# psipred/DMPfold2

Measured on AMD Instinct MI355X. Metric: structures/s at L=300, N_seq=2000, 10 iters+100 min, higher is better.
Workload: dtype f32 with full-width operands on the bf16 matrix cores (option precision = 2): convolution operands split exactly into 3 bf16 pieces (24 significand bits), the 6 piece products above 2^-24 accumulated in f32 by v_mfma_f32_32x32x16_bf16; vertical GRU the same way (3 bf16 pieces per operand, 6 products

## Files before the change

### dmpfold2_amd/csrc/conv_f16.h

```cpp
#pragma once
#include "common.h"
#include <cmath>
#include <vector>

namespace dmp {

typedef float ch_f32x16 __attribute__((ext_vector_type(16)));
typedef _Float16 ch_f16x8 __attribute__((ext_vector_type(8)));

#ifndef CH_PITCH_N
#define CH_PITCH_N 24
#endif
constexpr int CH_PITCH = CH_PITCH_N;
template <int NQ> struct ChShape {
  static constexpr int ROWS = 2 * NQ;
  static constexpr int HALO = ROWS + 4;
  static constexpr int RP = ROWS + 3;
  static constexpr int IN_SLOTS = 2 * 2 * HALO * CH_PITCH;
  static constexpr int IN_BYTES = IN_SLOTS * 16;
  static constexpr int PIECE = 2 * HALO * CH_PITCH;
};
constexpr int CH_HCOLS = 20;
constexpr int CH_WSLOT = 2 * 2 * 32;
constexpr int CH_WCOL = 5 * CH_WSLOT;
constexpr int CH_WBUF = 3 * CH_WSLOT;
template <int NQ> constexpr int convh_lds_bytes() { return ChShape<NQ>::IN_BYTES + 4 * CH_WBUF * 16; }
constexpr int CONVH_LDS_BYTES = convh_lds_bytes<8>();
inline int conv_split_rows(int tiles) { return 8 * tiles * tiles <= 256 ? 2 : 1; }
inline int conv_f16_grid(int tiles, int bands = 1) {
  const int nt = tiles * tiles * bands;
  return 8 * ((nt + 1) / 2);
}

__host__ __device__ inline uint16_t ch_f16_bits(float f) {
  const _Float16 h = (_Float16)f;
  return __builtin_bit_cast(uint16_t, h);
}
__host__ __device__ inline float ch_f16_f32(uint16_t b) {
  return (float)__builtin_bit_cast(_Float16, b);
}
__host__ __device__ inline void split2_f16(float x, uint16_t p[2]) {
  p[0] = ch_f16_bits(x);
  p[1] = ch_f16_bits(x - ch_f16_f32(p[0]));
}

inline float conv_weight_scale_f16(const float* w, size_t n) {
  float m = 0.f;
  for (size_t i = 0; i < n; ++i) m = std::fmax(m, std::fabs(w[i]));
  if (!(m > 0.f)) return 1.f;
  int e;
  std::frexp(m, &e);
  return std::ldexp(1.0f, 10 - e);
}

inline std::vector<uint16_t> pack_conv_weights_f16(const float* w, float scale) {
  const int tap_row[5] = {0, 2, 4, 1, 3};
  std::vector<uint16_t> q((size_t)4 * 8 * 25 * 4 * 2 * 2 * 32 * 8);
  for (int split = 0; split < 4; ++split)
    for (int g = 0; g < 8; ++g)
      for (int dx = 0; dx < 5; ++dx)
        for (int wave = 0; wave < 4; ++wave)
          for (int sl = 0; sl < 5; ++sl)
            for (int cg = 0; cg < 2; ++cg)
              for (int m = 0; m < 32; ++m)
                for (int e = 0; e < 8; ++e) {
                  const int oc = split * 128 + wave * 32 + m, ic = g * 16 + cg * 8 + e;
                  uint16_t p2[2];
                  split2_f16(scale * w[((size_t)oc * 128 + ic) * 25 + tap_row[sl] * 5 + dx], p2);
                  for (int p = 0; p < 2; ++p)
                    q[(((((((((size_t)split * 8 + g) * 5 + dx) * 4 + wave) * 5 + sl) * 2 + p) * 2 + cg) * 32 + m) * 8) + e] = p2[p];
                }
  return q;
}

#if defined(__HIPCC__) && defined(CONV_F16_KERNELS)
__device__ __forceinline__ void ch_dma16(const void* gsrc, unsigned lds_byte_addr) {
  unsigned keep;
  asm volatile("s_mov_b32 %0, m0\n\ts_mov_b32 m0, %2\n\ts_nop 0\n\tglobal_load_lds_dwordx4 %1, off\n\ts_mov_b32 m0, %0"
               : "=&s"(keep) : "v"(gsrc), "s"(lds_byte_addr) : "memory");
}
template <int N> __device__ __forceinline__ void ch_wait_vm() {
  asm volatile("s_waitcnt vmcnt(%0)" :: "n"(N) : "memory");
}
__device__ __forceinline__ ch_f32x16 ch_mfma(uint4 a, uint4 b, ch_f32x16 c) {
  return __builtin_amdgcn_mfma_f32_32x32x16_f16(__builtin_bit_cast(ch_f16x8, a),
                                                __builtin_bit_cast(ch_f16x8, b), c, 0, 0, 0);
}
__device__ __forceinline__ void ch_lane_pixel(int li, int& row, int& x) {
  const bool a = li < 4 || (li >= 12 && li < 16) || (li >= 20 && li < 28);
  row = a ? 0 : 1;
  if (a) x = li < 4 ? li : (li < 16 ? li - 8 : li - 12);
  else x = li < 12 ? li - 4 : (li < 20 ? li - 8 : li - 16);
}

template <int NQ, int NT, int PAR>
__device__ __forceinline__ void ch_column_pass(const uint4 (&a)[NT][2], const uint4* il, ch_f32x16 (&acc)[NQ]) {
  constexpr int PIECE = ChShape<NQ>::PIECE, RP = ChShape<NQ>::RP;
  uint4 bn0 = il[PAR * CH_PITCH], bn1 = il[PAR * CH_PITCH + PIECE];
#pragma unroll
  for (int r = PAR; r < RP; r += 2) {
    const uint4 b0 = bn0, b1 = bn1;
    if (r + 2 < RP) {
      bn0 = il[(r + 2) * CH_PITCH];
      bn1 = il[(r + 2) * CH_PITCH + PIECE];
    }
#pragma unroll
    for (int t = 0; t < NT; ++t) {
      const int q = (r - PAR - 2 * t) / 2;
      if (r - PAR - 2 * t >= 0 && q < NQ) acc[q] = ch_mfma(a[t][0], b1, acc[q]);
    }
#pragma unroll
    for (int t = 0; t < NT; ++t) {
      const int q = (r - PAR - 2 * t) / 2;
      if (r - PAR - 2 * t >= 0 && q < NQ) acc[q] = ch_mfma(a[t][1], b0, acc[q]);
    }
#pragma unroll
    for (int t = 0; t < NT; ++t) {
      const int q = (r - PAR - 2 * t) / 2;
      if (r - PAR - 2 * t >= 0 && q < NQ) acc[q] = ch_mfma(a[t][0], b0, acc[q]);
    }
  }
}

template <int NQ>
__global__ __launch_bounds__(256) __attribute__((amdgpu_waves_per_eu(3, 3))) void conv5x5_f16x3_kernel(const uint16_t* __restrict__ xs,
                                                               const uint16_t* __restrict__ wq,
                                                               const float* __restrict__ bias, float inv_scale,
                                                               int L, int P, int tiles, int nwork,
                                                               float* __restrict__ u, double* __restrict__ part) {
  using SH = ChShape<NQ>;
  constexpr int BANDS = 8 / NQ;
  extern __shared__ __attribute__((aligned(16))) unsigned char ch_smem[];
  const int id = blockIdx.x;
  const int xcd = id & 7, slot = id >> 3;
  const int ntiles = tiles * tiles * BANDS;
  const int tper = (ntiles + 1) >> 1;
  const int tile = (xcd >> 2) * tper + slot;
  const int split = xcd & 3;
  if (slot >= tper || tile >= ntiles) return;
  const int trow = tile / tiles, tcol = tile % tiles;
  const int ty0 = trow * SH::ROWS, tx0 = tcol * CONV_TILE;
  const int tid = threadIdx.x, lane = tid & 63;
  const int wave = __builtin_amdgcn_readfirstlane(tid >> 6);
  const int kk = lane >> 5, li = lane & 31;
  const int64_t PP = (int64_t)P * P;
  const int64_t half0 = ((int64_t)(trow / BANDS) * tiles + tcol) * 2 + (trow % BANDS);
  int prow, px;
  ch_lane_pixel(li, prow, px);
  if (BANDS == 2 && ty0 >= L) {
    if (li == 0 && prow == 0 && px == 0)
      for (int g4 = 0; g4 < 4; ++g4) {
        const int gch = split * 32 + wave * 8 + 2 * g4 + kk;
        part[(half0 * CW + gch) * 2 + 0] = 0.0;
        part[(half0 * CW + gch) * 2 + 1] = 0.0;
      }
    return;
  }

  const uint4* in_l = reinterpret_cast<const uint4*>(ch_smem);
  const uint4* w_l = reinterpret_cast<const uint4*>(ch_smem + SH::IN_BYTES) + wave * CH_WBUF;
  const unsigned lds_base = (unsigned)(size_t)(__attribute__((address_space(3))) unsigned char*)ch_smem;
  const unsigned w_lds_addr = lds_base + SH::IN_BYTES + wave * (CH_WBUF * 16);

  const uint4* xs4 = reinterpret_cast<const uint4*>(xs);
  auto in_src = [&](int e, int t) {
    const int s = e * 256 + t;
    const int sc = s < SH::IN_SLOTS ? s : 0;
    const int p = sc / SH::PIECE, r = sc % SH::PIECE;
    const int cg = r / (SH::HALO * CH_PITCH), r2 = r % (SH::HALO * CH_PITCH);
    const int yy = r2 / CH_PITCH;
    int xx = r2 % CH_PITCH;
    xx = xx < CH_HCOLS ? xx : 0;
    return (int)(((int64_t)(p * 16 + cg) * P + ty0 + yy) * P + tx0 + xx);
  };
  const uint4* wq4 = reinterpret_cast<const uint4*>(wq) + (int64_t)split * 8 * 5 * 4 * CH_WCOL +
                     (int64_t)wave * CH_WCOL + lane;
  const int b_base = (kk * SH::HALO + prow) * CH_PITCH + px;
  const int a_off = kk * 32 + li;

  ch_f32x16 acc[NQ];
#pragma unroll
  for (int q = 0; q < NQ; ++q)
#pragma unroll
    for (int r = 0; r < 16; ++r) acc[q][r] = 0.f;

  auto wdma = [&](int h) {
    const int odd = h & 1;
    const uint4* src = wq4 + (int64_t)(h >> 1) * 4 * CH_WCOL + odd * 3 * CH_WSLOT;
    if (odd) {
#pragma unroll
      for (int i = 0; i < 4; ++i) ch_dma16(src + 64 * i, w_lds_addr + 1024 * i);
    } else {
#pragma unroll
      for (int i = 0; i < 6; ++i) ch_dma16(src + 64 * i, w_lds_addr + 1024 * i);
    }
  };
  wdma(0);

  for (int g = 0; g < 8; ++g) {
    __syncthreads();
    {
      const uint4* src = xs4 + (int64_t)g * 2 * PP;
      const unsigned dst = lds_base + (wave * 64) * 16;
      int t = tid;
      asm volatile("" : "+v"(t));
#pragma unroll
      for (int e = 0; e < SH::IN_SLOTS / 256; ++e) ch_dma16(src + in_src(e, t), dst + e * 4096);
      if (wave * 64 < SH::IN_SLOTS % 256) ch_dma16(src + in_src(SH::IN_SLOTS / 256, t), dst + (SH::IN_SLOTS / 256) * 4096);
    }
    ch_wait_vm<0>();
    __syncthreads();
#pragma unroll 1
    for (int dx = 0; dx < 5; ++dx) {
      const uint4* il = in_l + b_base + dx;
      const int h0 = 2 * (g * 5 + dx);
      {
        ch_wait_vm<0>();
        uint4 a[3][2];
#pragma unroll
        for (int t = 0; t < 3; ++t) {
          a[t][0] = w_l[t * CH_WSLOT + a_off];
          a[t][1] = w_l[t * CH_WSLOT + 64 + a_off];
        }
        asm volatile("s_waitcnt lgkmcnt(0)" ::: "memory");
        wdma(h0 + 1);
        ch_column_pass<NQ, 3, 0>(a, il, acc);
      }
      {
        ch_wait_vm<0>();
        uint4 a[2][2];
#pragma unroll
        for (int t = 0; t < 2; ++t) {
          a[t][0] = w_l[t * CH_WSLOT + a_off];
          a[t][1] = w_l[t * CH_WSLOT + 64 + a_off];
        }
        asm volatile("s_waitcnt lgkmcnt(0)" ::: "memory");
        if (h0 + 2 < 80) wdma(h0 + 2);
        ch_column_pass<NQ, 2, 1>(a, il, acc);
      }
    }
  }

  const float* bsp = bias + split * 128 + wave * 32;
  const int64_t LL = (int64_t)L * L;
#pragma unroll
  for (int g4 = 0; g4 < 4; ++g4) {
    const int cl = 8 * g4 + 4 * kk;
    const int gch = split * 32 + wave * 8 + 2 * g4 + kk;
    const float b0 = bsp[cl], b1 = bsp[cl + 1], b2 = bsp[cl + 2], b3 = bsp[cl + 3];
#pragma unroll
    for (int hq = 0; hq < NQ / 4; ++hq) {
      float s1 = 0.f, s2 = 0.f;
#pragma unroll
      for (int q = 4 * hq; q < 4 * hq + 4; ++q) {
        float v = acc[q][4 * g4] * inv_scale + b0;
        v = fmaxf(v, acc[q][4 * g4 + 1] * inv_scale + b1);
        v = fmaxf(v, acc[q][4 * g4 + 2] * inv_scale + b2);
        v = fmaxf(v, acc[q][4 * g4 + 3] * inv_scale + b3);
        const int y = ty0 + 2 * q + prow, x = tx0 + px;
        if (y < L && x < L) {
          u[(int64_t)gch * LL + (int64_t)y * L + x] = v;
          s1 += v;
          s2 += v * v;
        }
      }
#pragma unroll
      for (int off = 16; off > 0; off >>= 1) {
        s1 += __shfl_xor(s1, off, 32);
        s2 += __shfl_xor(s2, off, 32);
      }
      if (li == 0) {
        part[((half0 + hq) * CW + gch) * 2 + 0] = (double)s1;
        part[((half0 + hq) * CW + gch) * 2 + 1] = (double)s2;
      }
    }
  }
}
#endif

}
```

Measured before the change: 4.384.

## Load conv weights directly into registers with software prefetch instead of LDS staging

Weights for the 5x5 conv were previously DMA'd from global memory into a per-wave LDS buffer and then read back into registers. Now each wave loads weight fragments straight from global memory into registers, prefetching the next half-column while the current column pass runs, with sched_barriers to keep that order. This frees the weight LDS region, precomputes the input-tile source offsets once, and sets launch bounds to 2 blocks per unit in place of the fixed waves-per-EU hint. The cost is higher register pressure and exposure to global memory latency on the weight loads if the prefetch does not cover it.

```diff
diff --git a/dmpfold2_amd/csrc/conv_f16.h b/dmpfold2_amd/csrc/conv_f16.h
--- a/dmpfold2_amd/csrc/conv_f16.h
+++ b/dmpfold2_amd/csrc/conv_f16.h
@@ -16,15 +16,15 @@
   static constexpr int ROWS = 2 * NQ;
   static constexpr int HALO = ROWS + 4;
   static constexpr int RP = ROWS + 3;
-  static constexpr int IN_SLOTS = 2 * 2 * HALO * CH_PITCH;
-  static constexpr int IN_BYTES = IN_SLOTS * 16;
   static constexpr int PIECE = 2 * HALO * CH_PITCH;
+  static constexpr int IN_SLOTS = 2 * PIECE;
+  static constexpr int IN_PAD = (IN_SLOTS + 63) / 64 * 64;
+  static constexpr int IN_BYTES = IN_PAD * 16;
 };
 constexpr int CH_HCOLS = 20;
 constexpr int CH_WSLOT = 2 * 2 * 32;
 constexpr int CH_WCOL = 5 * CH_WSLOT;
-constexpr int CH_WBUF = 3 * CH_WSLOT;
-template <int NQ> constexpr int convh_lds_bytes() { return ChShape<NQ>::IN_BYTES + 4 * CH_WBUF * 16; }
+template <int NQ> constexpr int convh_lds_bytes() { return ChShape<NQ>::IN_BYTES; }
 constexpr int CONVH_LDS_BYTES = convh_lds_bytes<8>();
 inline int conv_split_rows(int tiles) { return 8 * tiles * tiles <= 256 ? 2 : 1; }
 inline int conv_f16_grid(int tiles, int bands = 1) {
@@ -122,8 +122,16 @@
   }
 }
 
+template <int NT>
+__device__ __forceinline__ void ch_load_weights(const uint4* __restrict__ src, uint4 (&a)[NT][2]) {
+#pragma unroll
+  for (int t = 0; t < NT; ++t)
+#pragma unroll
+    for (int p = 0; p < 2; ++p) a[t][p] = src[t * CH_WSLOT + p * 64];
+}
+
 template <int NQ>
-__global__ __launch_bounds__(256) __attribute__((amdgpu_waves_per_eu(3, 3))) void conv5x5_f16x3_kernel(const uint16_t* __restrict__ xs,
+__global__ __launch_bounds__(256, 2) void conv5x5_f16x3_kernel(const uint16_t* __restrict__ xs,
                                                                const uint16_t* __restrict__ wq,
                                                                const float* __restrict__ bias, float inv_scale,
                                                                int L, int P, int tiles, int nwork,
@@ -158,25 +166,32 @@
   }
 
   const uint4* in_l = reinterpret_cast<const uint4*>(ch_smem);
-  const uint4* w_l = reinterpret_cast<const uint4*>(ch_smem + SH::IN_BYTES) + wave * CH_WBUF;
   const unsigned lds_base = (unsigned)(size_t)(__attribute__((address_space(3))) unsigned char*)ch_smem;
-  const unsigned w_lds_addr = lds_base + SH::IN_BYTES + wave * (CH_WBUF * 16);
 
   const uint4* xs4 = reinterpret_cast<const uint4*>(xs);
-  auto in_src = [&](int e, int t) {
-    const int s = e * 256 + t;
+  constexpr int NE = (SH::IN_PAD + 255) / 256;
+  int in_src[NE];
+#pragma unroll
+  for (int e = 0; e < NE; ++e) {
+    const int s = e * 256 + tid;
     const int sc = s < SH::IN_SLOTS ? s : 0;
     const int p = sc / SH::PIECE, r = sc % SH::PIECE;
     const int cg = r / (SH::HALO * CH_PITCH), r2 = r % (SH::HALO * CH_PITCH);
     const int yy = r2 / CH_PITCH;
     int xx = r2 % CH_PITCH;
     xx = xx < CH_HCOLS ? xx : 0;
-    return (int)(((int64_t)(p * 16 + cg) * P + ty0 + yy) * P + tx0 + xx);
+    in_src[e] = (int)(((int64_t)(p * 16 + cg) * P + ty0 + yy) * P + tx0 + xx);
+  }
+  auto tile_dma = [&](int g) {
+    const uint4* src = xs4 + (int64_t)g * 2 * PP;
+    const unsigned dst = lds_base + (wave * 64) * 16;
+#pragma unroll
+    for (int e = 0; e < SH::IN_PAD / 256; ++e) ch_dma16(src + in_src[e], dst + e * 4096);
+    if (wave * 64 < SH::IN_PAD % 256) ch_dma16(src + in_src[NE - 1], dst + (SH::IN_PAD / 256) * 4096);
   };
-  const uint4* wq4 = reinterpret_cast<const uint4*>(wq) + (int64_t)split * 8 * 5 * 4 * CH_WCOL +
-                     (int64_t)wave * CH_WCOL + lane;
+  const uint4* wcol = reinterpret_cast<const uint4*>(wq) + (int64_t)split * 8 * 5 * 4 * CH_WCOL +
+                      (int64_t)wave * CH_WCOL + lane;
   const int b_base = (kk * SH::HALO + prow) * CH_PITCH + px;
-  const int a_off = kk * 32 + li;
 
   ch_f32x16 acc[NQ];
 #pragma unroll
@@ -184,59 +199,32 @@
 #pragma unroll
     for (int r = 0; r < 16; ++r) acc[q][r] = 0.f;
 
-  auto wdma = [&](int h) {
-    const int odd = h & 1;
-    const uint4* src = wq4 + (int64_t)(h >> 1) * 4 * CH_WCOL + odd * 3 * CH_WSLOT;
-    if (odd) {
-#pragma unroll
-      for (int i = 0; i < 4; ++i) ch_dma16(src + 64 * i, w_lds_addr + 1024 * i);
-    } else {
-#pragma unroll
-      for (int i = 0; i < 6; ++i) ch_dma16(src + 64 * i, w_lds_addr + 1024 * i);
-    }
-  };
-  wdma(0);
+  uint4 ae[3][2], ao[2][2];
+  ch_load_weights<3>(wcol, ae);
+  __builtin_amdgcn_sched_barrier(0);
 
   for (int g = 0; g < 8; ++g) {
     __syncthreads();
-    {
-      const uint4* src = xs4 + (int64_t)g * 2 * PP;
-      const unsigned dst = lds_base + (wave * 64) * 16;
-      int t = tid;
-      asm volatile("" : "+v"(t));
-#pragma unroll
-      for (int e = 0; e < SH::IN_SLOTS / 256; ++e) ch_dma16(src + in_src(e, t), dst + e * 4096);
-      if (wave * 64 < SH::IN_SLOTS % 256) ch_dma16(src + in_src(SH::IN_SLOTS / 256, t), dst + (SH::IN_SLOTS / 256) * 4096);
-    }
+    tile_dma(g);
     ch_wait_vm<0>();
     __syncthreads();
+    const uint4* in_g = in_l + b_base;
 #pragma unroll 1
     for (int dx = 0; dx < 5; ++dx) {
-      const uint4* il = in_l + b_base + dx;
-      const int h0 = 2 * (g * 5 + dx);
+      const uint4* il = in_g + dx;
       {
-        ch_wait_vm<0>();
-        uint4 a[3][2];
-#pragma unroll
-        for (int t = 0; t < 3; ++t) {
-          a[t][0] = w_l[t * CH_WSLOT + a_off];
-          a[t][1] = w_l[t * CH_WSLOT + 64 + a_off];
-        }
-        asm volatile("s_waitcnt lgkmcnt(0)" ::: "memory");
-        wdma(h0 + 1);
-        ch_column_pass<NQ, 3, 0>(a, il, acc);
+        __builtin_amdgcn_sched_barrier(0);
+        ch_load_weights<2>(wcol + 3 * CH_WSLOT, ao);
+        __builtin_amdgcn_sched_barrier(0);
+        ch_column_pass<NQ, 3, 0>(ae, il, acc);
       }
       {
-        ch_wait_vm<0>();
-        uint4 a[2][2];
-#pragma unroll
-        for (int t = 0; t < 2; ++t) {
-          a[t][0] = w_l[t * CH_WSLOT + a_off];
-          a[t][1] = w_l[t * CH_WSLOT + 64 + a_off];
-        }
-        asm volatile("s_waitcnt lgkmcnt(0)" ::: "memory");
-        if (h0 + 2 < 80) wdma(h0 + 2);
-        ch_column_pass<NQ, 2, 1>(a, il, acc);
+        const uint4* wnext = wcol + (g * 5 + dx < 39 ? 4 * CH_WCOL : 0);
+        __builtin_amdgcn_sched_barrier(0);
+        ch_load_weights<3>(wnext, ae);
+        __builtin_amdgcn_sched_barrier(0);
+        ch_column_pass<NQ, 2, 1>(ao, il, acc);
+        wcol = wnext;
       }
     }
   }
```

New measurement: 4.383. No clear change (-0.0%).
